# DavidBluecame/libYafaRay

Hardware: AMD Instinct MI355X
Metric: Mrays/sec + Msamples/sec, 1920×1080×64spp path-trace at 1/2/4/8 GPUs (higher is better)
Workload: dtype f32

## Files before the change

### libyafaray_amd/csrc/devscene.h

```cpp
#pragma once
#include <cstdint>
#include <hip/hip_runtime.h>

namespace yafamd
{
struct DevStats;

struct RadGrid
{
	const uint32_t *start;
	const float4 *pos;
	const float4 *dir;
	float lo[3];
	float cell, inv_cell;
	int nx, ny, nz;
};

enum : uint32_t
{
	B_NONE = 0, B_SPECULAR = 1u << 0, B_GLOSSY = 1u << 1, B_DIFFUSE = 1u << 2, B_DISPERSIVE = 1u << 3,
	B_REFLECT = 1u << 4, B_TRANSMIT = 1u << 5, B_FILTER = 1u << 6, B_EMIT = 1u << 7, B_VOLUMETRIC = 1u << 8,
	B_ALL = B_SPECULAR | B_GLOSSY | B_DIFFUSE | B_DISPERSIVE | B_REFLECT | B_TRANSMIT | B_FILTER
};

// ... 161 lines not shown
	float shadow_bias, ray_min_dist;
	uint32_t base_offset, rr_seed;
	float clamp_samples;
	int aa_multipass;
	uint32_t pass_offset;
	const uint32_t *plist;
	int nee_all_count;
	int faure_bytes;
	int small_tables;

	const float4 *ph_pos;
	const float4 *ph_dir;
	const float *ph_colb;
	const uint4 *pk_nodes;
	uint2 *pk_stack;
	int n_photons, pm_paths, pm_search, pm_stack;
	float pm_radius2;
	const int *ph_lights;
	const float *light_cdf;
	const float *light_func;
	float light_inv_integral;
	int n_ph_lights;
	const float4 *cph_pos;
	const float4 *cph_dir;
	const float *cph_colb;
	const uint4 *cpk_nodes;
	int caus_map, c_photons, c_paths, c_search;
	float c_radius2;
	int gather_on;
	int fg_on, fg_samples, fg_bounces;
	int fg_pass_samples;
	float fg_min_pathlen;
	float fg_lookup_rad;
	float fg_i_scale;
	const float4 *rph_pos;
	const float4 *rph_dir;
	const float *rph_colb;
	const uint4 *rpk_nodes;
	int n_rphotons;
	int rpk_lds;
	RadGrid rgrid;

	int has_attr, n_textures;
	const float4 *prim_attr;
	const float4 *texels;
	const DevTexture *textures;
	const DevNode *shader_nodes;

	int ext, tree, raydepth, cur_level;
	int max_add_depth;
	int bg_transp_refract;
	int tr_shad, s_depth;
	int do_ao, ao_samples;
	float ao_dist;
	float ao_col[3];
	struct DevStats *stats;
	int trace_stats;
	int crop_x0, crop_y0;
	int show_map;
	uint32_t node_base;
	uint32_t spawn_cap;
	float4 *node_own;
	int2 *node_child;
	float4 *node_w;
	float4 *spawn_o, *spawn_d;
	uint4 *spawn_pr;
	uint32_t *spawn_count;
	uint32_t *lpc;
	int lpc_mode;
	uint32_t *dfr_kind;
	float4 *dfr_pp;
	float4 *dfr_wo;
	float4 *dfr_a;
	float4 *dfr_emit;
	uint2 *dfr_pix;
	uint32_t *dfr_last;
	const uint32_t *dfr_seg_off;
	uint32_t dfr_cap;
	int nee_pm16;
	int w_live;
	int no_lean;
	int has_mesh_light;
	int fg_probe;
};

struct DevFilm
{
	float table[256];
	float filterw, table_scale;
	int reach_fwd, reach_back;
	int width, height, spp, tile;
	int multipass;
	uint32_t sample_offset;
	const uint32_t *tile_rank;
	int ntx;
	int partial;
	int crop_x0, crop_y0;
};

enum : int
{
	LK_BARYCENTRIC = 0, LK_DIFFUSE_COLOR, LK_MAT_INDEX_ABS, LK_MAT_INDEX_NORM, LK_MIST, LK_NORMAL_GEOM, LK_NORMAL_SMOOTH,
	LK_OBJ_INDEX_ABS, LK_OBJ_INDEX_NORM, LK_UV, LK_ZDEPTH_ABS, LK_ZDEPTH_NORM, LK_COUNT
};

struct DevLayers
{
	int n;
	int kind[LK_COUNT];
	const float4 *prim_attr;
	const float *mat_index;
	const int2 *obj_seg;
	int n_obj_seg;
	int n_prims, n_mats;
	float mat_highest, obj_highest;
	const float *depth;
	float4 *rec;
	float4 *albedo;
};

struct DevPaths
{
	float4 *thr;
	float4 *col;
	float4 *pcol;
	float4 *pwo;
	float4 *pend_thr;
	float4 *pend_emit;
	float4 *v0p;
	float4 *v0wo;
	uint4 *pr;
	float4 *csmp;
	float *nee;
	float *nee_aw;
	uint8_t *occ;
	float4 *ts;
	float4 *v0attr;
};

struct DevQueues
{
	int *slot;
	float *ray_o;
	float *ray_d;
	float2 *ray_tt;
	float tmin_dflt;
	float *hit_t;
	int *hit_prim;
	float4 *sh_o;
	float4 *sh_d;
	int *sh_idx;
	float2 *ts_hit;
	int *ts_n;
	float4 *sattr;
	const uint32_t *perm;
	int trace_part;
	int nee_grid;
};

enum : int
{
	TRACE_BOTH = 0,
	TRACE_CLOSEST = 1,
	TRACE_SHADOW = 2,
};

// ... 105 lines not shown
```

### libyafaray_amd/csrc/kernels.hip

```cpp

#include <hip/hip_runtime.h>
#include <cstdlib>
#include <string>
#include "devmath.h"
#include "photonheap.h"
#include "devscene.h"
#include "texeval.h"

namespace yafamd
{

#ifndef YAF_TRACE_BLOCK
#define YAF_TRACE_BLOCK 128
#endif
#ifndef YAF_SHADE_MIN_WAVES
#define YAF_SHADE_MIN_WAVES 4
#endif
#ifndef YAF_SHADE_LEAN_WAVES
#define YAF_SHADE_LEAN_WAVES 4
#endif
#ifndef YAF_SHADE_PREFETCH
#define YAF_SHADE_PREFETCH 1
#endif
constexpr int kTraceBlock = YAF_TRACE_BLOCK;
// ... 136 lines not shown
	__builtin_nontemporal_store(v, p);
#else
	*p = v;
#endif
}

__device__ __forceinline__ bool loadQRay(const DevQueues &Q, uint32_t i, V3 &o, V3 &d, float &tmin, float &tmax_w)
{
	const F3 dd = rayLd3(Q.ray_d, i);
	const F3 oo = rayLd3(Q.ray_o, i);
	d = v3(dd.x, dd.y, dd.z);
	o = v3(oo.x, oo.y, oo.z);
	if(dd.x != dd.x) return false;
	if(Q.ray_tt)
	{
		const float2 tt = Q.ray_tt[i];
		tmin = tt.x;
		tmax_w = tt.y;
	}
	else
	{
		tmin = Q.tmin_dflt;
		tmax_w = -1.f;
	}
	return true;
}
typedef float f32x3a4_t __attribute__((ext_vector_type(3))) __attribute__((aligned(4)));
__device__ __forceinline__ void storeQRay(const DevQueues &Q, uint32_t i, V3 o, V3 d)
{
#if YAF_NT_STORE2
	f32x3a4_t vo, vd;
	vo.x = o.x; vo.y = o.y; vo.z = o.z;
	vd.x = d.x; vd.y = d.y; vd.z = d.z;
	__builtin_nontemporal_store(vo, reinterpret_cast<f32x3a4_t *>(Q.ray_o + 3 * (size_t)i));
	__builtin_nontemporal_store(vd, reinterpret_cast<f32x3a4_t *>(Q.ray_d + 3 * (size_t)i));
#else
	reinterpret_cast<F3 *>(Q.ray_o)[i] = F3{o.x, o.y, o.z};
	reinterpret_cast<F3 *>(Q.ray_d)[i] = F3{d.x, d.y, d.z};
#endif
}
__device__ __forceinline__ void stStoreF3(float4 *base, uint32_t k, C3 c)
{
#if YAF_NT_STORE
	f32x3a4_t v;
	v.x = c.r; v.y = c.g; v.z = c.b;
	__builtin_nontemporal_store(v, reinterpret_cast<f32x3a4_t *>(reinterpret_cast<float *>(base) + 3 * (size_t)k));
#else
	reinterpret_cast<F3 *>(base)[k] = F3{c.r, c.g, c.b};
#endif
}
__device__ __forceinline__ void storeQNoRay(const DevQueues &Q, uint32_t i)
{
	Q.ray_d[3 * (size_t)i] = __builtin_nanf("");
}

constexpr uint32_t kPmSBits = 20, kPmLBits = 11;
__device__ __forceinline__ bool neePm8(const DevScene &S)
{
	return !S.nee_pm16 && (uint32_t)S.spp < (1u << kPmSBits) && S.n_lights <= (1 << kPmLBits);
}
typedef uint32_t u32x2_t __attribute__((ext_vector_type(2)));
#ifdef YAF_CHECKED
__device__ uint32_t g_nee_pm_err = 0;
#define NEE_PM_GUARD(cond) do { if(!(cond)) atomicCAS(&g_nee_pm_err, 0u, (uint32_t)__LINE__); } while(0)
#else
#define NEE_PM_GUARD(cond) do {} while(0)
#endif
__device__ __forceinline__ void neePmStore(const DevScene &S, uint4 *pm, uint32_t j, uint32_t offset, uint32_t sample_idx, uint32_t mode_l)
{
	if(neePm8(S))
	{
		NEE_PM_GUARD(sample_idx - S.base_offset - S.pass_offset < (uint32_t)S.spp);
		u32x2_t w;
		w.x = offset;
		w.y = (sample_idx - S.base_offset - S.pass_offset) | ((mode_l & 1u) << kPmSBits) | ((mode_l >> 8) << (kPmSBits + 1));
#if YAF_NT_STORE2
		__builtin_nontemporal_store(w, reinterpret_cast<u32x2_t *>(pm) + j);
#else
		reinterpret_cast<u32x2_t *>(pm)[j] = w;
#endif
	}
	else stStore2(&pm[j], make_uint4(offset, sample_idx, mode_l, 0u));
}
__device__ __forceinline__ uint4 neePmLoad(const DevScene &S, const uint4 *pm, uint32_t j)
{
	if(neePm8(S))
	{
		const uint2 w = reinterpret_cast<const uint2 *>(pm)[j];
		const uint32_t rel = w.y & ((1u << kPmSBits) - 1u);
		return make_uint4(w.x, S.base_offset + S.pass_offset + rel, ((w.y >> kPmSBits) & 1u) | ((w.y >> (kPmSBits + 1)) << 8), 0u);
	}
	return pm[j];
}

struct SegLoop
{
	uint32_t s, r, nb;
};
__device__ __forceinline__ SegLoop segLoop(uint32_t n_seg)
{
	SegLoop L;
	L.s = blockIdx.x % n_seg;
	L.r = blockIdx.x / n_seg;
	L.nb = (gridDim.x - L.s + n_seg - 1) / n_seg;
	return L;
}

#ifdef YAF_PHASE_TIMING
__device__ unsigned long long g_phase[16];
#define PHASE_DECL uint64_t ph_t = clock64(); uint64_t ph_acc[8] = {0, 0, 0, 0, 0, 0, 0, 0};
#define PHASE(k) do { const uint64_t t_ = clock64(); ph_acc[k] += t_ - ph_t; ph_t = t_; } while(0)
#define PHASE_FLUSH do { if(laneId() == 0) for(int k_ = 0; k_ < 8; ++k_) atomicAdd(&g_phase[k_], (unsigned long long)ph_acc[k_]); } while(0)
#else
#define PHASE_DECL
#define PHASE(k)
#define PHASE_FLUSH
#endif

struct SampleCoord { int x, y, s; };

__device__ SampleCoord sampleCoord(const DevJob *jobs, int n_jobs, int width, int tile, int spp, uint64_t sid)
{
	int j = 0, hi = n_jobs - 1;
	while(j < hi)
	{
		const int mid = (j + hi + 1) >> 1;
		if(jobs[mid].sample_base <= sid) j = mid;
		else hi = mid - 1;
	}
	const DevJob job = jobs[j];
	const uint64_t local = sid - job.sample_base;
	const uint32_t pix = (uint32_t)(local / (uint64_t)spp);
	const int s = (int)(local % (uint64_t)spp);
	const int bh = job.y1 - job.y0;
	const uint32_t per_tile = (uint32_t)(tile * bh);
	const int tx = (int)(pix / per_tile);
	const int tw = min(tile, width - tx * tile);
	const uint32_t l = pix - (uint32_t)tx * per_tile;
	SampleCoord c;
	c.x = tx * tile + (int)(l % (uint32_t)tw);
	c.y = job.y0 + (int)(l / (uint32_t)tw);
	c.s = s;
	return c;
}

__device__ __forceinline__ float biasDist(int bias, float r)
{
	if(bias == 1) return sqrtf(sqrtf(r) * r);
	if(bias == 2) return sqrtf(1.f - r * r);
	return sqrtf(r);
}

__device__ __forceinline__ void shirleyDisk(float r_1, float r_2, float &u, float &v)
{
	float phi = 0.f, r = 0.f;
	const float a = 2.f * r_1 - 1.f, b = 2.f * r_2 - 1.f;
	if(a > -b)
	{
		if(a > b) { r = a; phi = x87mul(kDivPiBy4, b / a); }
		else { r = b; phi = x87mul(kDivPiBy4, 2.f - a / b); }
	}
	else
	{
		if(a < b) { r = -a; phi = x87mul(kDivPiBy4, 4.f + b / a); }
		else
		{
			r = -b;
			phi = (b != 0) ? x87mul(kDivPiBy4, 6.f - a / b) : 0.f;
		}
	}
	u = r * fcos(phi);
	v = r * fsin(phi);
}

// ... 2028 lines not shown
}

__device__ __forceinline__ float ldsDim(const DevScene &S, int dim, uint32_t n)
{
	const uint4 fd = S.faure_dim[dim];
	UDiv dv;
	dv.m = fd.z;
	dv.sh = fd.w;
	return (float)lowDiscrepancy(S.faure + fd.y, fd.x, dv, S.faure_inv[dim], n);
}

__device__ __forceinline__ void copy16(uint4 *dst, const void *src, int n)
{
	const uint4 *s4 = reinterpret_cast<const uint4 *>(src);
	for(int k = threadIdx.x; k < n; k += blockDim.x) dst[k] = s4[k];
}

#ifndef YAF_STAGE_MATS
#define YAF_STAGE_MATS 1
#endif
constexpr size_t kStageMatsMax = 8192;
__host__ __device__ inline bool stageMatsOnly(const DevScene &S, bool small)
{
	return YAF_STAGE_MATS && !small && (size_t)S.n_mats * sizeof(DevMaterial) <= kStageMatsMax;
}
__host__ __device__ inline size_t shadeLdsBytes(const DevScene &S, bool small)
{
	size_t b = 50 * 16 + 25 * 16 + (size_t)S.faure_bytes;
	if(small) b += (size_t)S.n_mats * sizeof(DevMaterial) + (size_t)S.n_tris * 16;
	else if(stageMatsOnly(S, small)) b += (size_t)S.n_mats * sizeof(DevMaterial);
	return b;
}

template<bool SMALL>
__device__ __forceinline__ DevScene stageTables(const DevScene &G, uint4 *smem)
{
	DevScene S = G;
	uint4 *p = smem;
	copy16(p, G.faure_dim, 50);
	S.faure_dim = p;
	p += 50;
	copy16(p, G.faure_inv, 25);
	S.faure_inv = reinterpret_cast<const double *>(p);
	p += 25;
	if(SMALL)
	{
		const int nm = G.n_mats * (int)(sizeof(DevMaterial) / 16);
		copy16(p, G.mats, nm);
		S.mats = reinterpret_cast<const DevMaterial *>(p);
		p += nm;
		copy16(p, G.prim_ng, G.n_tris);
		S.prim_ng = reinterpret_cast<const float4 *>(p);
		p += G.n_tris;
	}
	else if(stageMatsOnly(G, false))
	{
		const int nm = G.n_mats * (int)(sizeof(DevMaterial) / 16);
		copy16(p, G.mats, nm);
		S.mats = reinterpret_cast<const DevMaterial *>(p);
		p += nm;
	}
	copy16(p, G.faure, G.faure_bytes / 16);
	S.faure = reinterpret_cast<const uint8_t *>(p);
	__syncthreads();
	return S;
}

struct ShadeArgs
{
	DevScene S;
	DevPaths Pc;
	DevPaths Pn;
	DevQueues Q;
	DevQueues Qn;
	DevNeeQueue N;
	DevNeeQueue G;
	DevCounters cnt;
	DevCounters cnt_next;
	float4 *samples;
	const DevJob *jobs;
	int n_jobs;
	uint64_t chunk_base;
};

__device__ __forceinline__ void writeSampleAt(const ShadeArgs &A, const SampleCoord &sc, C3 col, float alpha)
{
	if(alpha > 1.f) alpha = 1.f;
	A.samples[((size_t)sc.y * A.S.width + sc.x) * A.S.spp + sc.s] = f4(col, alpha);
}

__device__ __forceinline__ void writeSample(const ShadeArgs &A, uint32_t sid, C3 col, float alpha)
{
	writeSampleAt(A, sampleAt(A.S, A.jobs, A.n_jobs, A.chunk_base + (uint64_t)sid), col, alpha);
}

__device__ __forceinline__ Surf surfFromPrim(const DevScene &S, V3 p, int prim)
{
	Surf s;
	s.p = p;
	const float4 g = S.prim_ng[prim];
	s.ng = xyz(g);
	s.n = s.ng;
	coordsSystem(s.n, s.nu, s.nv);
	s.mat = __float_as_int(g.w);
	s.flags = S.mats[s.mat].bsdf_flags;
	const DevMaterial &m = S.mats[s.mat];
	s.dcol = C3{m.diffuse[0], m.diffuse[1], m.diffuse[2]};
	s.drefl = 1.f;
	s.sigma = 0.f;
	return s;
}

__device__ void spawnSpecular(const DevScene &S, const DevMaterial &m, const Surf &sp, V3 wo, uint32_t node, uint2 pix, uint2 rng,
                              int additional_depth)
{
	int2 child = make_int2(-1, -1);
	const int level = S.cur_level + 1;
	additional_depth = max(additional_depth, m.add_depth);
	if((sp.flags & (B_SPECULAR | B_FILTER)) && level <= S.raydepth + additional_depth && level < 20)
	{
		const SpecOut so = matSpecular(m, sp, wo);
		for(int k = 0; k < 2; ++k)
		{
			const bool want = k == 0 ? so.refl : so.refr;
			if(!want) continue;
			const uint32_t idx = atomicAdd(&S.spawn_count[0], 1u);
			if(idx >= S.spawn_cap) { atomicOr(&S.spawn_count[1], 1u); continue; }
			V3 from = sp.p;
			const V3 dir = k == 0 ? so.rdir : so.tdir;
			if(k == 1 && m.tbias > 0.f)
			{
				float f = m.tbias;
				if(m.sd_flags & SD_TBIAS_MULT) f *= (float)level;
				from = sp.p + dir * f;
			}
			S.spawn_o[idx] = f4(from, S.ray_min_dist);
			S.spawn_d[idx] = f4(dir, -1.f - (float)additional_depth);
			S.spawn_pr[idx] = make_uint4(pix.x, pix.y, rng.x ^ (0x9e3779b9u * (uint32_t)(2 * level + k + 1)), rng.y + 1u + (uint32_t)k);
			S.node_w[S.node_base + idx] = f4(k == 0 ? so.rcol : so.tcol, 0.f);
			if(k == 0) child.x = (int)(S.node_base + idx);
			else child.y = (int)(S.node_base + idx);
		}
	}
	S.node_child[node] = child;
}

template<bool SMALL, bool EXT, bool FUSED = false, bool LEAN = false, bool DEFER = false>
__global__ void __launch_bounds__(kShadeBlock, EXT ? 1 : (LEAN ? YAF_SHADE_LEAN_WAVES : YAF_SHADE_MIN_WAVES)) k_shade(ShadeArgs A)
{
	extern __shared__ uint4 shade_smem[];
	DevScene S_ = stageTables<SMALL>(A.S, shade_smem);
	if constexpr(LEAN)
	{
		S_.integrator = INT_PATH;
		S_.path_samples = 1;
		S_.do_ao = 0;
		S_.caus_map = 0;
		S_.show_map = 0;
		S_.gather_on = 0;
		S_.n_photons = 0;
		S_.fg_on = 0;
		S_.tree = 0;
		S_.has_attr = 0;
	}
	const DevScene S = S_;
	const bool ATTR = EXT && S.has_attr != 0;
// ... 755 lines not shown
			const uint32_t h = lo <= hi ? 1u : 0u;
			child[k] = __float_as_int(lane4(cf, k));
			const int count = __float_as_int(lane4(kf, k));
			const uint32_t inner = child[k] >= 0 ? 1u : 0u;
			key[k] = (h & inner) ? lo : inf;
			s4[k] = ~child[k] - acc;
			acc += (h & (inner ^ 1u)) ? count : 0;
			e4[k] = acc;
		}
		bool done = false;
		for(int i = 0; i < e4[3]; ++i)
		{
			const int q = i + (i < e4[0] ? s4[0] : i < e4[1] ? s4[1] : i < e4[2] ? s4[2] : s4[3]);
			if(STATS) TRACE_STAT(++tests);
			const float4 *tp = C.tris + 3 * q;
			const float4 ta = tp[0], tb = tp[1], tc = tp[2];
			const float t = triTest(ta, tb, tc, o, d, t_best);
			if(t == -1.f) continue;
			const int prim = __float_as_int(tb.w);
			if(any)
			{
				if(t < tmax && t >= 0.f) { t_best = t; prim_best = prim; done = true; break; }
			}
			else if(t >= tmin && (t < t_best || (t == t_best && prim_best >= 0 && prim < prim_best)))
			{
				t_best = t;
				prim_best = prim;
			}
		}
		if(!done)
		{
			cswap(key[0], child[0], key[1], child[1]);
			cswap(key[2], child[2], key[3], child[3]);
			cswap(key[0], child[0], key[2], child[2]);
			cswap(key[1], child[1], key[3], child[3]);
			cswap(key[1], child[1], key[2], child[2]);
			if(key[3] < inf) { C.stack[sp * STRIDE + lane] = child[3]; ++sp; }
			if(key[2] < inf) { C.stack[sp * STRIDE + lane] = child[2]; ++sp; }
			if(key[1] < inf) { C.stack[sp * STRIDE + lane] = child[1]; ++sp; }
			int next = key[0] < inf ? child[0] : -1;
			if(next < 0 && sp > 0)
			{
				--sp;
				next = C.stack[sp * STRIDE + lane];
			}
			node = next;
			done = next < 0;
		}
		if(done)
		{
			if(any) occ[cur] = prim_best >= 0 ? 1 : 0;
			else
			{
				hit_t = t_best;
				hit_prim = prim_best;
			}
			node = -1;
		}
	}
}

struct NeeArgs
{
	DevScene S;
	DevNeeQueue N;
	DevPaths Pn;
	DevQueues Qn;
	DevCounters cnt_next;
	int stack_depth;
};

__host__ __device__ inline size_t neeTraceLdsBytes(const DevScene &S, int stack_depth)
{
	return shadeLdsBytes(S, true) + (size_t)(S.node_f4 * S.n_nodes + 3 * S.n_tris) * 16 + (size_t)stack_depth * kShadeBlock * 4 +
	       (size_t)kShadeBlock * S.nee_k * 32;
}

#ifndef YAF_NEE_MIN_WAVES
#define YAF_NEE_MIN_WAVES 4
#endif
#ifndef YAF_NEE_LEAN_WAVES
#define YAF_NEE_LEAN_WAVES 4
#endif
#ifndef YAF_NEE_PREFETCH
#define YAF_NEE_PREFETCH 0
#endif
template<bool SMALL, bool EXT, bool TR = false, bool TSTATS = false, bool LEAN = false>
__global__ void __launch_bounds__(kShadeBlock, EXT ? 1 : (LEAN ? YAF_NEE_LEAN_WAVES : YAF_NEE_MIN_WAVES)) k_nee(NeeArgs A)
{
	extern __shared__ uint4 shade_smem[];
	DevScene S_ = stageTables<SMALL>(A.S, shade_smem);
	if constexpr(LEAN)
	{
		S_.do_ao = 0;
		S_.tr_shad = 0;
		S_.has_attr = 0;
	}
	const DevScene S = S_;
	const bool ATTR = EXT && S.has_attr != 0;
	TraceCtx C;
	C.wave_base = waveBase();
	float4 *rec = nullptr;
	if(TR)
	{
		float4 *lds_nodes = reinterpret_cast<float4 *>(shade_smem) + shadeLdsBytes(S, SMALL) / 16;
		float4 *lds_tris = lds_nodes + S.node_f4 * S.n_nodes;
		int *stack = reinterpret_cast<int *>(lds_tris + 3 * S.n_tris);
		rec = reinterpret_cast<float4 *>(stack + A.stack_depth * kShadeBlock) + 2 * threadIdx.x * S.nee_k;
		for(int k = threadIdx.x; k < S.node_f4 * S.n_nodes; k += blockDim.x) lds_nodes[k] = A.S.nodes[k];
		for(int k = threadIdx.x; k < 3 * S.n_tris; k += blockDim.x) lds_tris[k] = A.S.tris[k];
		__syncthreads();
		C.nodes = lds_nodes;
		C.tris = lds_tris;
		C.stack = stack;
		C.lds_depth = A.stack_depth;
		C.spill = nullptr;
		C.spill_stride = 0;
	}
	__shared__ uint32_t s_count;
	for(uint32_t seg = blockIdx.x; seg < S.n_seg; seg += gridDim.x)
	{
	uint32_t n_shadow = 0, n_dummy = 0, visits = 0, tests = 0;
	if(threadIdx.x == 0) s_count = 0;
	__syncthreads();
	ShadeOut out;
	out.sh_count = &s_count;
	out.sh_base = seg * S.cap_s;
	out.Qn = A.Qn;
	out.idx_in_o = !S.tr_shad;
	const uint32_t n_req = A.cnt_next.n_nee[seg];
	const uint32_t n_slots = A.cnt_next.n_active[seg];
	const uint32_t a0 = seg * S.cap_a;
	const int K = S.nee_k;
	const uint32_t stride = blockDim.x;
#if YAF_NEE_PREFETCH
	float4 wk_n = make_float4(0.f, 0.f, 0.f, 0.f);
	F3 o_n{0.f, 0.f, 0.f};
	uint4 pm_n = make_uint4(0u, 0u, 0u, 0u);
	if(threadIdx.x < n_slots)
	{
		wk_n = A.N.wo_k[a0 + threadIdx.x];
		o_n = reinterpret_cast<const F3 *>(A.Qn.ray_o)[a0 + threadIdx.x];
		pm_n = neePmLoad(S, A.N.pix_mode, a0 + threadIdx.x);
	}
#endif
	for(uint32_t base_j = 0; base_j < n_slots; base_j += stride)
	{
		const uint32_t j = a0 + base_j + threadIdx.x;
		float4 wk = make_float4(0.f, 0.f, 0.f, 0.f);
		V3 p = v3(0.f, 0.f, 0.f);
		uint4 pm = make_uint4(0u, 0u, 0u, 0u);
		bool live = base_j + threadIdx.x < n_slots;
#if YAF_NEE_PREFETCH
		if(live)
		{
			wk = wk_n;
			p = v3(o_n.x, o_n.y, o_n.z);
			pm = pm_n;
			live = !(wk.x != wk.x);
		}
		if(base_j + stride + threadIdx.x < n_slots)
		{
			wk_n = A.N.wo_k[j + stride];
			o_n = reinterpret_cast<const F3 *>(A.Qn.ray_o)[j + stride];
			pm_n = neePmLoad(S, A.N.pix_mode, j + stride);
		}
#else
		if(live)
		{
			wk = A.N.wo_k[j];
			const F3 o = reinterpret_cast<const F3 *>(A.Qn.ray_o)[j];
			p = v3(o.x, o.y, o.z);
			pm = neePmLoad(S, A.N.pix_mode, j);
			live = !(wk.x != wk.x);
		}
#endif
		Surf sp;
		sp.p = v3(0.f, 0.f, 0.f); sp.n = sp.ng = sp.nu = sp.nv = sp.p; sp.mat = 0; sp.flags = 0;
		sp.dcol = c3(0.f); sp.drefl = 1.f; sp.sigma = 0.f;
		if(live) sp = surfFromPrim(S, p, __float_as_int(wk.w));
		if(ATTR && live) applyAttr(sp, A.N.attr[2 * (size_t)j], A.N.attr[2 * (size_t)j + 1]);
		const V3 wo = xyz(wk);
		const int e0 = (int)j * K;
		const bool all = live && (pm.z & 1u);
		const bool one = live && !(pm.z & 1u);
		const uint32_t lnum = pm.z >> 8;
		if constexpr(TR)
		{
			if(live)
				for(int e = 0; e < K; ++e) rec[2 * e + 1] = make_float4(0.f, 0.f, 0.f, 0.f);
			const PathShadows rs{rec, e0};
			for(int l = 0; l < S.n_lights; ++l)
			{
				const bool mine = all || (one && lnum == (uint32_t)l);
				if(!__any(mine)) continue;
				neeLight<EXT>(S, S.lights[l], S.mats[sp.mat], sp, wo, (uint32_t)l, pm.y, pm.x, mine, e0 + (all ? (int)S.lights[l].nee_base : 0),
				              neeHbm(A.Pn), A.Pn.occ, rs);
			}
			float t_dummy;
			int p_dummy;
			if(__any(live))
				traceLaneRays<TSTATS, kShadeBlock>(C, rec, A.Pn.occ + e0, K, live, false, v3(0.f, 0.f, 0.f), v3(0.f, 0.f, 1.f), 0.f, 0.f, t_dummy,
				                                  p_dummy, visits, tests, n_dummy, n_shadow);
			continue;
		}
		if(__any(all))
		{
			for(int l = 0; l < S.n_lights; ++l)
				neeLight<EXT, ShadeOut, NeeHbm, LEAN>(S, S.lights[l], S.mats[sp.mat], sp, wo, (uint32_t)l, pm.y, pm.x, all,
				         e0 + (int)S.lights[l].nee_base, neeHbm(A.Pn), A.Pn.occ, out, S.tr_shad ? A.Pn.ts : nullptr);
			if(S.do_ao)
				aoSamples<EXT>(S, S.mats[sp.mat], sp, wo, pm.y, pm.x, all, e0 + S.nee_all_count, neeHbm(A.Pn), A.Pn.occ, out,
				               S.tr_shad ? A.Pn.ts : nullptr);
		}
		if(__any(one))
		{
			for(int l = 0; l < S.n_lights; ++l)
			{
				const bool mine = one && lnum == (uint32_t)l;
				if(!__any(mine)) continue;
				neeLight<EXT, ShadeOut, NeeHbm, LEAN>(S, S.lights[l], S.mats[sp.mat], sp, wo, (uint32_t)l, pm.y, pm.x, mine, e0, neeHbm(A.Pn), A.Pn.occ, out,
				              S.tr_shad ? A.Pn.ts : nullptr);
			}
		}
	}
	if(TR)
	{
		for(int off = 32; off > 0; off >>= 1) n_shadow += __shfl_down(n_shadow, off);
		if(laneId() == 0 && n_shadow) atomicAdd(&s_count, n_shadow);
	}
	__syncthreads();
	if(threadIdx.x == 0)
	{
		A.cnt_next.n_shadow[seg] = TR ? 0u : s_count;
		if(S.stats)
		{
			S.stats[seg].nee_requests += n_req;
			if(TR) S.stats[seg].shadow_rays += s_count;
		}
	}
	if(TR && TSTATS && S.stats)
	{
		for(int off = 32; off > 0; off >>= 1)
		{
			visits += __shfl_down(visits, off);
			tests += __shfl_down(tests, off);
		}
		if(laneId() == 0)
		{
			atomicAdd(&S.stats[seg].node_visits, (unsigned long long)visits);
			atomicAdd(&S.stats[seg].tri_tests, (unsigned long long)tests);
		}
	}
	}
}

struct DfrArgs
{
	DevScene S;
// ... 2721 lines not shown
					if(v.w != 0.f) path_col = path_col + rgb(v);
				}
			}
		}
		const C3 fg = path_col / (float)B.n_sampl;
		const uint4 cb = A.G.pix_mode[j];
		const C3 col = C3{__uint_as_float(cb.x), __uint_as_float(cb.y), __uint_as_float(cb.z)} + fg;
		A.G.pix_mode[j] = make_uint4(__float_as_uint(col.r), __float_as_uint(col.g), __float_as_uint(col.b), cb.w);
	}
}

}

using namespace yafamd;

extern "C" {

int yafamd_trace_block() { return kTraceBlock; }

int yafamd_shade_fused() { return kShadeFused ? 1 : 0; }
int yafamd_shade_fused_for(const DevScene *S)
{
	if(S->ext) return 0;
	if(kShadeFused) return 1;
	return (YAF_FUSE_LEAN && S->integrator == INT_PATH && S->path_samples <= 1 && !S->do_ao && !S->caus_map && !S->gather_on && !S->show_map &&
	        S->n_photons == 0 && !S->tree && !S->has_attr && !S->no_lean && !S->tr_shad && !S->has_mesh_light) ? 1 : 0;
}

int yafamd_experiments() { return kExperiments ? 1 : 0; }

#ifndef YAF_DEVICE_BUILD
#define YAF_DEVICE_BUILD "arch=? extra=[?] (built outside csrc/Makefile)"
#endif
const char *yafamd_device_build() { return YAF_DEVICE_BUILD
#ifdef YAF_PHASE_TIMING
	" phase-timing"
#endif
	; }

int yafamd_phase_cycles(unsigned long long *out, int n, int reset)
{
#ifdef YAF_PHASE_TIMING
	unsigned long long h[16];
	if(hipMemcpyFromSymbol(h, HIP_SYMBOL(g_phase), sizeof(h)) != hipSuccess) return 0;
	for(int k = 0; k < n && k < 16; ++k) out[k] = h[k];
	if(reset)
	{
		const unsigned long long z[16] = {};
		if(hipMemcpyToSymbol(HIP_SYMBOL(g_phase), z, sizeof(z)) != hipSuccess) return 0;
	}
	return 16;
#else
	(void)out; (void)n; (void)reset;
	return 0;
#endif
}

int yafamd_trace_blocks_per_cu(int lds_scene, int wide, size_t dyn_lds)
{
	int nb = 0;
	hipError_t e;
	if(wide == 8) e = hipOccupancyMaxActiveBlocksPerMultiprocessor(&nb, k_trace<false, true, false, true, false, false, true>, kTraceBlock, dyn_lds);
	else if(lds_scene) e = wide ? hipOccupancyMaxActiveBlocksPerMultiprocessor(&nb, k_trace<true, true, false>, kTraceBlock, dyn_lds)
	                       : hipOccupancyMaxActiveBlocksPerMultiprocessor(&nb, k_trace<true, false, false>, kTraceBlock, dyn_lds);
	else e = wide ? hipOccupancyMaxActiveBlocksPerMultiprocessor(&nb, k_trace<false, true, false>, kTraceBlock, dyn_lds)
	              : hipOccupancyMaxActiveBlocksPerMultiprocessor(&nb, k_trace<false, false, false>, kTraceBlock, dyn_lds);
	return e == hipSuccess ? nb : 0;
}

int yafamd_path_blocks_per_cu(const DevScene *S, int stack_depth)
{
	int nb = 0;
#ifdef YAF_EXPERIMENTS
	if(hipOccupancyMaxActiveBlocksPerMultiprocessor(&nb, k_path<false>, kTraceBlock, pathLdsBytes(*S, stack_depth)) != hipSuccess) nb = 0;
#else
	(void)S; (void)stack_depth;
#endif
	return nb;
}

int yafamd_nee_blocks_per_cu()
{
	int nb = 0;
	if(hipOccupancyMaxActiveBlocksPerMultiprocessor(&nb, (k_nee<true, false>), kShadeBlock, 8192) != hipSuccess) nb = 0;
	return nb;
}

int yafamd_shade_blocks_per_cu()
{
	int nb = 0;
	if(hipOccupancyMaxActiveBlocksPerMultiprocessor(&nb, (k_shade<true, false>), kShadeBlock, 8192) != hipSuccess) nb = 0;
	return nb;
}

hipError_t yafamd_launch_camera(const DevScene *S, const DevPaths *P, const DevQueues *Q, const DevCounters *cnt,
                                const DevJob *jobs, int n_jobs, uint64_t chunk_base, int n, hipStream_t st)
{
	if(n <= 0) return hipSuccess;
	const int threads = max(n, (int)S->n_seg);
	hipLaunchKernelGGL(k_camera, dim3((threads + 255) / 256), dim3(256), 0, st, *S, *P, *Q, *cnt, jobs, n_jobs, chunk_base, n);
	return hipGetLastError();
}

hipError_t yafamd_launch_trace(const DevScene *S, const DevQueues *Q, const DevCounters *cnt, const DevPaths *P,
                               DevStats *stats, int stack_depth, int *spill, int grid, hipStream_t st)
{
	const size_t stack_bytes = (size_t)stack_depth * kTraceBlock * sizeof(int);
	const bool wide = S->node_f4 == 8;
	const size_t lds_scene = S->scene_in_lds ? (size_t)(S->node_f4 * S->n_nodes + 3 * S->n_tris) * sizeof(float4)
	                                         : (wide ? (size_t)S->lds_top * kTopStride * sizeof(float4) : 0);
	const size_t bytes = stack_bytes + lds_scene;
	if(S->nodes8 && !S->scene_in_lds && !S->tr_shad)
	{
		const size_t bytes8 = stack_bytes + (size_t)S->lds_top8 * kTop8Stride * sizeof(float4);
		if(S->trace_stats)
			hipLaunchKernelGGL((k_trace<false, true, false, true, true, false, true>), dim3(grid), dim3(kTraceBlock), bytes8, st, *S, *Q, *cnt, *P, stats,
			                   stack_depth, spill);
		else
			hipLaunchKernelGGL((k_trace<false, true, false, true, false, false, true>), dim3(grid), dim3(kTraceBlock), bytes8, st, *S, *Q, *cnt, *P, stats,
			                   stack_depth, spill);
		return hipGetLastError();
	}
#ifdef YAF_EXPERIMENTS
	if(S->brute && !S->tr_shad && S->n_tris <= kBruteTris)
	{
		hipLaunchKernelGGL(k_trace_brute, dim3(grid), dim3(kTraceBlock), 0, st, *S, *Q, *cnt, *P, stats);
		return hipGetLastError();
	}
#endif
#define YAF_TRACE_LAUNCH(L, W, T, SP) hipLaunchKernelGGL((k_trace<L, W, T, SP>), dim3(grid), dim3(kTraceBlock), bytes, st, *S, *Q, *cnt, *P, stats, stack_depth, spill)
	const bool nospill = spill == nullptr;
	if(S->tr_shad)
	{
		if(S->scene_in_lds)
		{
			if(nospill) { if(wide) YAF_TRACE_LAUNCH(true, true, true, false); else YAF_TRACE_LAUNCH(true, false, true, false); }
			else if(wide) YAF_TRACE_LAUNCH(true, true, true, true);
			else YAF_TRACE_LAUNCH(true, false, true, true);
		}
		else if(wide) YAF_TRACE_LAUNCH(false, true, true, true);
		else YAF_TRACE_LAUNCH(false, false, true, true);
	}
	else if(S->scene_in_lds)
	{
#ifdef YAF_EXPERIMENTS
		if(nospill && wide && S->ray_sort)
		{
			if(S->trace_stats)
				hipLaunchKernelGGL((k_trace<true, true, false, false, true, true>), dim3(grid), dim3(kTraceBlock), bytes, st, *S, *Q, *cnt, *P, stats,
				                   stack_depth, spill);
			else
				hipLaunchKernelGGL((k_trace<true, true, false, false, false, true>), dim3(grid), dim3(kTraceBlock), bytes, st, *S, *Q, *cnt, *P, stats,
				                   stack_depth, spill);
		}
		else
#endif
		if(nospill && wide && !S->trace_stats)
			hipLaunchKernelGGL((k_trace<true, true, false, false, false>), dim3(grid), dim3(kTraceBlock), bytes, st, *S, *Q, *cnt, *P, stats,
			                   stack_depth, spill);
		else if(nospill) { if(wide) YAF_TRACE_LAUNCH(true, true, false, false); else YAF_TRACE_LAUNCH(true, false, false, false); }
		else if(wide) YAF_TRACE_LAUNCH(true, true, false, true);
		else YAF_TRACE_LAUNCH(true, false, false, true);
	}
#ifdef YAF_EXPERIMENTS
	else if(wide && S->ray_sort)
	{
		if(S->trace_stats)
// ... 143 lines not shown
}

hipError_t yafamd_launch_surface(const DevScene *S, const DevQueues *Q, const DevCounters *cnt, hipStream_t st)
{
	hipLaunchKernelGGL(k_surface, dim3(S->n_seg), dim3(kShadeBlock), 0, st, *S, *Q, *cnt);
	return hipGetLastError();
}

hipError_t yafamd_launch_tshadow(const DevScene *S, const DevQueues *Q, const DevCounters *cnt, const DevPaths *P, hipStream_t st)
{
	hipLaunchKernelGGL(k_tshadow, dim3(S->n_seg), dim3(kShadeBlock), 0, st, *S, *Q, *cnt, *P);
	return hipGetLastError();
}

int yafamd_path_eligible(const DevScene *S, int stack_depth, int spill)
{
	return (kExperiments && !S->ext && !S->tree && !S->tr_shad && !S->has_attr && !S->do_ao && !S->gather_on && !S->caus_map && S->integrator != INT_PHOTON &&
	        S->scene_in_lds && S->node_f4 == 8 && !spill && S->small_tables && S->nee_k >= 1 && S->nee_k <= kPathMaxK && !S->brute &&
	        pathLdsBytes(*S, stack_depth) <= 64 * 1024)
	           ? 1
	           : 0;
}

hipError_t yafamd_launch_path(const DevScene *S, float4 *samples, const DevJob *jobs, int n_jobs, uint64_t chunk_base, uint32_t n,
                              uint32_t *next, int stack_depth, int grid, hipStream_t st)
{
	if(!yafamd_path_eligible(S, stack_depth, 0)) return hipErrorInvalidValue;
	if(n == 0) return hipSuccess;
	PathArgs A;
	A.S = *S;
	A.samples = samples;
	A.jobs = jobs;
	A.n_jobs = n_jobs;
	A.chunk_base = chunk_base;
	A.n = n;
	A.next = next;
	A.stack_depth = stack_depth;
#ifdef YAF_EXPERIMENTS
	const size_t lds = pathLdsBytes(*S, stack_depth);
	if(S->trace_stats) hipLaunchKernelGGL(k_path<true>, dim3(grid), dim3(kTraceBlock), lds, st, A);
	else hipLaunchKernelGGL(k_path<false>, dim3(grid), dim3(kTraceBlock), lds, st, A);
	return hipGetLastError();
#else
	(void)grid; (void)st;
	return hipErrorInvalidValue;
#endif
}

int yafamd_nee_trace_eligible(const DevScene *S, int stack_depth)
{
	return (kExperiments && !S->ext && !S->tr_shad && !S->has_attr && S->scene_in_lds && S->node_f4 == 8 && S->small_tables && S->nee_k >= 1 &&
	        S->nee_k <= kPathMaxK && !S->brute && neeTraceLdsBytes(*S, stack_depth) <= 64 * 1024)
	           ? 1
	           : 0;
}

hipError_t yafamd_launch_nee(const DevScene *S, const DevNeeQueue *N, const DevPaths *Pn, const DevQueues *Qn,
                             const DevCounters *cnt_next, int stack_depth, hipStream_t st)
{
	NeeArgs A;
	A.S = *S;
	A.N = *N;
	A.Pn = *Pn;
	A.Qn = *Qn;
	A.cnt_next = *cnt_next;
	const size_t lds = shadeLdsBytes(*S, S->small_tables != 0);
	A.stack_depth = stack_depth;
	const int grid = (Qn->nee_grid > 0 && Qn->nee_grid < (int)S->n_seg) ? Qn->nee_grid : (int)S->n_seg;
#ifdef YAF_EXPERIMENTS
	if(stack_depth > 0 && yafamd_nee_trace_eligible(S, stack_depth))
	{
		if(S->trace_stats) hipLaunchKernelGGL((k_nee<true, false, true, true>), dim3(grid), dim3(kShadeBlock), neeTraceLdsBytes(*S, stack_depth), st, A);
		else hipLaunchKernelGGL((k_nee<true, false, true>), dim3(grid), dim3(kShadeBlock), neeTraceLdsBytes(*S, stack_depth), st, A);
		return hipGetLastError();
	}
#endif
	if(S->ext)
	{
		if(S->small_tables) hipLaunchKernelGGL((k_nee<true, true>), dim3(grid), dim3(kShadeBlock), lds, st, A);
		else hipLaunchKernelGGL((k_nee<false, true>), dim3(grid), dim3(kShadeBlock), lds, st, A);
	}
	else if(!S->do_ao && !S->tr_shad && !S->has_mesh_light && !S->no_lean)
	{
		if(S->small_tables) hipLaunchKernelGGL((k_nee<true, false, false, false, true>), dim3(grid), dim3(kShadeBlock), lds, st, A);
		else hipLaunchKernelGGL((k_nee<false, false, false, false, true>), dim3(grid), dim3(kShadeBlock), lds, st, A);
	}
	else if(S->small_tables) hipLaunchKernelGGL((k_nee<true, false>), dim3(grid), dim3(kShadeBlock), lds, st, A);
	else hipLaunchKernelGGL((k_nee<false, false>), dim3(grid), dim3(kShadeBlock), lds, st, A);
	return hipGetLastError();
}

hipError_t yafamd_photon_emit(const DevScene *S, const PhotonState *P, const PhotonSet *L, uint32_t n_photons, uint32_t h0, uint32_t n_local,
                              int max_bounces, hipStream_t st)
{
	PhotonArgs A;
	A.S = *S;
	A.P = *P;
	A.L = *L;
	A.n_photons = n_photons;
	A.h0 = h0;
	A.n_local = n_local;
	A.max_bounces = max_bounces;
	A.bounce = 0;
	A.cur = 0;
	A.stack_depth = 0;
	A.spill = nullptr;
	if(n_local == 0) return hipSuccess;
	hipLaunchKernelGGL(k_photon_emit, dim3((n_local + 255) / 256), dim3(256), 0, st, A);
	return hipGetLastError();
}

hipError_t yafamd_photon_bounce(const DevScene *S, const PhotonState *P, const PhotonSet *L, uint32_t n_photons, uint32_t h0,
                                uint32_t n_local, int max_bounces, int bounce, int cur, int stack_depth, int *spill, int grid, hipStream_t st)
{
	PhotonArgs A;
	A.S = *S;
	A.P = *P;
	A.L = *L;
	A.n_photons = n_photons;
	A.h0 = h0;
	A.n_local = n_local;
	A.max_bounces = max_bounces;
	A.bounce = bounce;
	A.cur = cur;
	A.stack_depth = stack_depth;
	A.spill = spill;
	if((uint32_t)grid != P->n_segs) return hipErrorInvalidValue;
	const size_t stack_bytes = (size_t)stack_depth * kTraceBlock * sizeof(int);
	if(S->scene_in_lds)
	{
		const size_t bytes = stack_bytes + (size_t)(S->node_f4 * S->n_nodes + 3 * S->n_tris) * sizeof(float4);
		const bool ns = spill == nullptr;
		if(S->ext)
		{
			if(S->node_f4 == 8)
			{
				if(ns) hipLaunchKernelGGL((k_photon_bounce<true, true, true, false>), dim3(grid), dim3(kTraceBlock), bytes, st, A);
				else hipLaunchKernelGGL((k_photon_bounce<true, true, true>), dim3(grid), dim3(kTraceBlock), bytes, st, A);
			}
			else hipLaunchKernelGGL((k_photon_bounce<true, false, true>), dim3(grid), dim3(kTraceBlock), bytes, st, A);
		}
		else if(S->node_f4 == 8)
		{
			if(ns) hipLaunchKernelGGL((k_photon_bounce<true, true, false, false>), dim3(grid), dim3(kTraceBlock), bytes, st, A);
			else hipLaunchKernelGGL((k_photon_bounce<true, true, false>), dim3(grid), dim3(kTraceBlock), bytes, st, A);
		}
		else hipLaunchKernelGGL((k_photon_bounce<true, false, false>), dim3(grid), dim3(kTraceBlock), bytes, st, A);
	}
	else if(S->ext)
	{
		if(S->node_f4 == 8) hipLaunchKernelGGL((k_photon_bounce<false, true, true>), dim3(grid), dim3(kTraceBlock), stack_bytes, st, A);
		else hipLaunchKernelGGL((k_photon_bounce<false, false, true>), dim3(grid), dim3(kTraceBlock), stack_bytes, st, A);
	}
	else if(S->node_f4 == 8) hipLaunchKernelGGL((k_photon_bounce<false, true, false>), dim3(grid), dim3(kTraceBlock), stack_bytes, st, A);
	else hipLaunchKernelGGL((k_photon_bounce<false, false, false>), dim3(grid), dim3(kTraceBlock), stack_bytes, st, A);
	return hipGetLastError();
}

hipError_t yafamd_photon_compact(const PhotonState *P, uint32_t *scratch_counts, uint32_t *total_dev, float4 *pos, float4 *dir, float *colb,
                                 hipStream_t st)
{
	const uint32_t nb = (P->n_local + 1023u) / 1024u;
	if(nb == 0) return hipSuccess;
	hipLaunchKernelGGL(k_photon_count, dim3(nb), dim3(256), 0, st, P->dep_flag, P->n_local, P->n_slot_rows, scratch_counts);
	hipLaunchKernelGGL(k_photon_scan, dim3(1), dim3(1024), 0, st, scratch_counts, nb, total_dev);
	hipLaunchKernelGGL(k_photon_scatter, dim3(nb), dim3(1024), 0, st, *P, (const uint32_t *)scratch_counts, pos, dir, colb);
	return hipGetLastError();
// ... 264 lines not shown
```

### libyafaray_amd/csrc/render.cc

```cpp
#include "render.h"
#include "devmath.h"
#include "photonfile.h"

#include <hip/hip_runtime.h>
#include <rccl/rccl.h>

#include <algorithm>
#include <array>
#include <chrono>
#include <cmath>
#include <cstdlib>
#include <cstring>
#include <future>
#include <mutex>
#include <sstream>
#include <unordered_map>

using namespace yafamd;

extern "C" {
hipError_t yafamd_launch_camera(const DevScene *S, const DevPaths *P, const DevQueues *Q, const DevCounters *cnt,
                                const DevJob *jobs, int n_jobs, uint64_t chunk_base, int n, hipStream_t st);
hipError_t yafamd_launch_surface(const DevScene *S, const DevQueues *Q, const DevCounters *cnt, hipStream_t st);
hipError_t yafamd_launch_tshadow(const DevScene *S, const DevQueues *Q, const DevCounters *cnt, const DevPaths *P, hipStream_t st);
// ... 1999 lines not shown
			const char *we = std::getenv("YAFARAY_AMD_GATHER_WALK");
			const uint32_t exact = (yafamd_experiments() && we && std::string(we) == "bound") ? 0u : 1u;
			glog = GatherLogDesc{d.g_log.p, (uint32_t *)d.g_log_n.p, cap, (uint32_t)seg_cap, 0u, split, exact, nullptr};
			const int lv = yafamd_walk_lds_levels(d.pm_stack), deep = std::max(1, d.pm_stack) - lv;
			if(deep > 0)
			{
				if(!ensure(log_, d.walk_spill, (size_t)deep * yafamd_walk_threads(&S) * 4)) return false;
				glog.spill = (uint32_t *)d.walk_spill.p;
			}
			walk_gather = true;
		}
	}
	const bool fg_paths = yafamd_fg_paths_eligible(&S) != 0;
	bool ray_bin = false;
	if(const char *e = std::getenv("YAFARAY_AMD_RAY_BIN"); e && *e == '1' && S.nodes8 && !S.scene_in_lds && !S.tr_shad && R <= 1024)
	{
		const size_t n = (size_t)R * S.cap_a;
		size_t tb = 0;
		HIPCHECK(yafamd_ray_bin(nullptr, nullptr, (uint32_t)R, S.cap_a, nullptr, nullptr, nullptr, nullptr, nullptr, nullptr, nullptr, &tb, d.stream));
		if(!ensure(log_, d.bin_keys, n * 4) || !ensure(log_, d.bin_keys2, n * 4) || !ensure(log_, d.bin_iota, n * 4) || !ensure(log_, d.bin_perm, n * 4) ||
		   !ensure(log_, d.bin_tmp, tb))
			return false;
		ray_bin = true;
	}
	FgBatch fgb{};
	auto fgPrepare = [&]() -> bool {
		const int ns = S.fg_pass_samples > 0 ? S.fg_pass_samples : std::max(1, S.fg_samples);
		const int nt = std::max(0, S.fg_bounces) + 1;
		const size_t per_pos = (size_t)R * (size_t)ns * (16 + 48 + 16 * (size_t)nt);
		size_t cap_max = std::max<size_t>(1, ((size_t)6 << 30) / per_pos);
		if(const char *e = getenv("YAFARAY_AMD_FG_BATCH"); e && atoi(e) > 0) cap_max = std::min(cap_max, (size_t)atoi(e));
		const size_t nb = ((size_t)S.cap_a + cap_max - 1) / cap_max;
		const size_t seg_cap = std::max<size_t>(1, ((size_t)S.cap_a + nb - 1) / std::max<size_t>(1, nb));
		const size_t paths = (size_t)R * seg_cap * (size_t)ns;
		if(!ensure(log_, d.fg_terms, paths * 16) || !ensure(log_, d.fg_longs, paths * 48) || !ensure(log_, d.fg_long_terms, paths * 16 * (size_t)nt) ||
		   !ensure(log_, d.fg_long_count, (size_t)R * 4))
			return false;
		fgb = FgBatch{0u, (uint32_t)seg_cap, ns, nt, (float4 *)d.fg_terms.p, (float4 *)d.fg_longs.p, (float4 *)d.fg_long_terms.p,
		              (uint32_t *)d.fg_long_count.p, (uint32_t)(seg_cap * (size_t)ns)};
		return true;
	};
	if(!ensure(log_, d.counters, 2 * 4 * R * sizeof(uint32_t))) return false;
	if(!ensure(log_, d.stats, sizeof(DevStats) * 2 * (size_t)d.trace_grid)) return false;
	HIPCHECK(hipMemsetAsync(d.counters.p, 0, 2 * 4 * R * sizeof(uint32_t), d.stream));
	HIPCHECK(hipMemsetAsync(d.stats.p, 0, sizeof(DevStats) * 2 * (size_t)d.trace_grid, d.stream));
	DevCounters cnt[2];
	for(int q = 0; q < 2; ++q)
	{
		uint32_t *base_q = (uint32_t *)d.counters.p + (size_t)q * 4 * R;
		cnt[q].n_active = base_q;
		cnt[q].n_shadow = base_q + R;
		cnt[q].n_nee = base_q + 2 * R;
		cnt[q].n_gather = base_q + 3 * R;
	}
	DevStats *dstats = (DevStats *)d.stats.p;
	S.stats = dstats;
	int nee_trace_stack = 0;
	{
		const char *ne = std::getenv("YAFARAY_AMD_NEE_TRACE");
		if(yafamd_experiments() && ne && std::string(ne) == "1" && d.lds_stack >= d.stack_depth) nee_trace_stack = d.lds_stack;
	}
	bool overlap = rp.device_sharers <= 1;
	int ov_nee_grid = std::max(1, (int)S.n_seg / 2), ov_trace_grid = std::max((int)S.n_seg, std::min(2 * (int)S.n_seg, d.trace_grid));
	if(const char *e = std::getenv("YAFARAY_AMD_OVERLAP"); e && *e) overlap = *e != '0';
	if(const char *e = std::getenv("YAFARAY_AMD_OVERLAP_NEE_GRID"); e && atoi(e) > 0) ov_nee_grid = atoi(e);
	if(const char *e = std::getenv("YAFARAY_AMD_OVERLAP_TRACE_GRID"); e && atoi(e) > 0)
		ov_trace_grid = (int)S.n_seg * std::max(1, std::min(atoi(e), d.trace_grid) / (int)S.n_seg);
	overlap = overlap && S.scene_in_lds && !S.ray_sort && !S.brute && !ray_bin && !S.tree && !S.tr_shad && !S.has_attr && nee_trace_stack == 0;
	bool ov_shadow = true;
	int ov_shadow_grid = d.trace_grid;
	if(const char *e = std::getenv("YAFARAY_AMD_OVERLAP_SHADOW"); e && *e) ov_shadow = *e != '0';
	if(const char *e = std::getenv("YAFARAY_AMD_OVERLAP_SHADOW_GRID"); e && atoi(e) > 0)
		ov_shadow_grid = (int)S.n_seg * std::max(1, std::min(atoi(e), d.trace_grid) / (int)S.n_seg);
	ov_shadow = ov_shadow && overlap && d.spill.p == nullptr;
	bool lpc_on = S.integrator == INT_PATH && S.n_lights > 1 && !S.tree && (rp.shard_world <= 1 || group_render);
	if(const char *lp = std::getenv("YAFARAY_AMD_LIGHT_PICK"); lp && std::string(lp) == "hash") lpc_on = false;
	lpc_carry_ = 0;
	S.lpc = nullptr;
	S.lpc_mode = 0;
	S.nee_pm16 = 0;
	if(const char *e = std::getenv("YAFARAY_AMD_NEE_PM16"); e && *e == '1') S.nee_pm16 = 1;
	if(const char *e = std::getenv("YAFARAY_AMD_W_LIVE"); e && *e == '1') S.w_live = 1;
	S.no_lean = 0;
	S.fg_probe = 0;
	if(const char *e = std::getenv("YAFARAY_AMD_FG_PROBE"); e && *e) S.fg_probe = atoi(e);
	if(const char *e = std::getenv("YAFARAY_AMD_SHADE_LEAN"); e && *e == '0') S.no_lean = 1;
	int path_grid = 0;
	if(!lpc_on)
	{
		const char *pe = std::getenv("YAFARAY_AMD_PATH");
		const bool on = yafamd_experiments() && pe && std::string(pe) == "mega";
		if(on && yafamd_path_eligible(&S, d.lds_stack, d.lds_stack < d.stack_depth ? 1 : 0))
		{
			path_grid = std::min(d.trace_grid, d.n_cu * std::max(1, yafamd_path_blocks_per_cu(&S, d.lds_stack)));
			if(const char *e = getenv("YAFARAY_AMD_PATH_GRID")) path_grid = std::min(d.trace_grid, std::max(1, atoi(e)));
			if(!ensure(log_, d.path_next, 16)) return false;
		}
	}
	const int n_paths = std::max(1, S.path_samples);
	const int iters = (S.integrator == INT_PATH) ? 2 + n_paths * (S.bounces + 2) : 3;

	auto ensureEvents = [&](size_t need) -> bool {
		while(d.ev_pool.size() < need)
		{
			hipEvent_t e;
			HIPCHECK(hipEventCreate(&e));
			d.ev_pool.push_back(e);
		}
		return true;
	};
	if(!ensureEvents(2)) return false;
	HIPCHECK(hipEventRecord(d.ev_pool[0], d.stream));
	DevStats *run_stats = dstats;
	auto iterate = [&](uint64_t base) -> bool {
		int cur = 0;
		const bool count_run = S.lpc_mode == 1;
		bool closest_done = false;
		for(int it = 0; it < iters; ++it)
		{
			DevQueues qc = d.Q[cur];
			if(it != 0 || (S.cur_level == 0 && !S.cam.ray_tt)) qc.ray_tt = nullptr;
			qc.tmin_dflt = it == 0 ? 0.f : S.ray_min_dist;
			qc.perm = nullptr;
			qc.trace_part = closest_done ? TRACE_SHADOW : TRACE_BOTH;
			const bool join_pending = closest_done && ov_shadow;
			closest_done = false;
			if(ray_bin && it >= 1 && !count_run)
			{
				size_t tb = d.bin_tmp.bytes;
				HIPCHECK(yafamd_ray_bin(&qc, &cnt[cur], S.n_seg, S.cap_a, d.scene_lo, d.scene_hi, (uint32_t *)d.bin_keys.p, (uint32_t *)d.bin_keys2.p,
				                        (uint32_t *)d.bin_iota.p, (uint32_t *)d.bin_perm.p, d.bin_tmp.p, &tb, d.stream));
				qc.perm = (const uint32_t *)d.bin_perm.p;
			}
			if(join_pending)
			{
				bool ok = [&]() -> bool {
					PROF(KK_TRACE, yafamd_launch_trace(&S, &qc, &cnt[cur], &d.P[cur], run_stats + d.trace_grid, d.lds_stack, nullptr, ov_shadow_grid,
					                                    d.stream));
					HIPCHECK(hipStreamWaitEvent(d.stream, d.ev_join, 0));
					return true;
				}();
				if(!ok)
				{
					(void)hipStreamSynchronize(d.side);
					return false;
				}
			}
			else
				PROF(KK_TRACE, yafamd_launch_trace(&S, &qc, &cnt[cur], &d.P[cur], run_stats, d.lds_stack, (int *)d.spill.p,
				                                    S.tr_shad ? d.trace_grid_bvh4 : d.trace_grid, d.stream));
			if(S.tr_shad && !count_run) PROF(KK_TSHADOW, yafamd_launch_tshadow(&S, &qc, &cnt[cur], &d.P[cur], d.stream));
			if(S.has_attr) PROF(KK_SURFACE, yafamd_launch_surface(&S, &qc, &cnt[cur], d.stream));
			if(S.lpc_mode == 3)
				HIPCHECK(yafamd_dfr_segoff(&cnt[cur], S.n_seg, (uint32_t *)d.dfr_segoff.p, (uint32_t *)d.dfr_misc.p, S.dfr_cap,
				                           (uint32_t *)d.dfr_misc.p + 1, (uint32_t *)d.dfr_its.p, d.stream));
			PROF(KK_SHADE, yafamd_launch_shade(&S, &d.P[cur], &d.P[cur ^ 1], &qc, &d.Q[cur ^ 1], &d.N, &d.G, &cnt[cur], &cnt[cur ^ 1],
			                             (float4 *)d.samples.p, (const DevJob *)d.jobs.p, n_jobs, base, d.stream));

			const bool dl_pipeline = S.integrator != INT_PATH;
			if(S.gather_on && !count_run && (!dl_pipeline || it == 1 || (S.show_map && it == 0)))
			{
				if(S.fg_on && fg_paths)
				{
					if(!fgPrepare()) return false;
					for(uint32_t j0 = 0; j0 < S.cap_a; j0 += fgb.seg_cap)
					{
// ... 981 lines not shown
```

Before: 2169.

## Prefetch NEE slot inputs into LDS via global_load_lds DMA in lean k_nee

Replaces the compile-time register prefetch in the lean NEE kernel with an asynchronous global-to-LDS DMA prefetch (global_load_lds) of wo_k, ray origins and pixel-mode words for the next iteration. Each wave gets a 3 KB LDS staging area, and the loads for iteration j+stride are issued while the current slot is shaded, so global latency is hidden without holding extra registers. This costs 6 KB more LDS per block, which may lower occupancy. The path is on by default and can be turned off with an environment variable.

```diff
diff --git a/libyafaray_amd/csrc/devscene.h b/libyafaray_amd/csrc/devscene.h
--- a/libyafaray_amd/csrc/devscene.h
+++ b/libyafaray_amd/csrc/devscene.h
@@ -267,6 +267,7 @@
 	int no_lean;
 	int has_mesh_light;
 	int fg_probe;
+	int nee_pf_lds;
 };
 
 struct DevFilm
diff --git a/libyafaray_amd/csrc/kernels.hip b/libyafaray_amd/csrc/kernels.hip
--- a/libyafaray_amd/csrc/kernels.hip
+++ b/libyafaray_amd/csrc/kernels.hip
@@ -242,14 +242,14 @@
 	}
 	else stStore2(&pm[j], make_uint4(offset, sample_idx, mode_l, 0u));
 }
+__device__ __forceinline__ uint4 neePmWide(const DevScene &S, uint2 w)
+{
+	const uint32_t rel = w.y & ((1u << kPmSBits) - 1u);
+	return make_uint4(w.x, S.base_offset + S.pass_offset + rel, ((w.y >> kPmSBits) & 1u) | ((w.y >> (kPmSBits + 1)) << 8), 0u);
+}
 __device__ __forceinline__ uint4 neePmLoad(const DevScene &S, const uint4 *pm, uint32_t j)
 {
-	if(neePm8(S))
-	{
-		const uint2 w = reinterpret_cast<const uint2 *>(pm)[j];
-		const uint32_t rel = w.y & ((1u << kPmSBits) - 1u);
-		return make_uint4(w.x, S.base_offset + S.pass_offset + rel, ((w.y >> kPmSBits) & 1u) | ((w.y >> (kPmSBits + 1)) << 8), 0u);
-	}
+	if(neePm8(S)) return neePmWide(S, reinterpret_cast<const uint2 *>(pm)[j]);
 	return pm[j];
 }
 
@@ -2444,6 +2444,22 @@
 	int n_jobs;
 	uint64_t chunk_base;
 };
+
+template<int SIZE>
+__device__ __forceinline__ void ldsDma(const void *src, char *wave_dst)
+{
+	static_assert(SIZE == 4 || SIZE == 12 || SIZE == 16, "global_load_lds_dword / x3 / x4");
+	const auto *g = (const __attribute__((address_space(1))) void *)src;
+	auto *l = (__attribute__((address_space(3))) void *)wave_dst;
+	if constexpr(SIZE == 4) __builtin_amdgcn_global_load_lds(g, l, 4, 0, 0);
+	else if constexpr(SIZE == 12) __builtin_amdgcn_global_load_lds(g, l, 12, 0, 0);
+	else __builtin_amdgcn_global_load_lds(g, l, 16, 0, 0);
+}
+__device__ __forceinline__ void ldsDmaLanded() { asm volatile("s_waitcnt vmcnt(0)" ::: "memory"); }
+__device__ __forceinline__ void ldsReadsRetired() { asm volatile("s_waitcnt lgkmcnt(0)" ::: "memory"); }
+constexpr uint32_t kPfPitch12 = 16;
+constexpr uint32_t kNeePfWk = 0, kNeePfO = 1024, kNeePfPm = 2048, kNeePfWave = 3072;
+constexpr size_t kNeePfBytes = (size_t)(kShadeBlock / 64) * kNeePfWave;
 
 __device__ __forceinline__ void writeSampleAt(const ShadeArgs &A, const SampleCoord &sc, C3 col, float alpha)
 {
@@ -3365,12 +3381,10 @@
 #ifndef YAF_NEE_LEAN_WAVES
 #define YAF_NEE_LEAN_WAVES 4
 #endif
-#ifndef YAF_NEE_PREFETCH
-#define YAF_NEE_PREFETCH 0
-#endif
-template<bool SMALL, bool EXT, bool TR = false, bool TSTATS = false, bool LEAN = false>
+template<bool SMALL, bool EXT, bool TR = false, bool TSTATS = false, bool LEAN = false, bool PFL = false>
 __global__ void __launch_bounds__(kShadeBlock, EXT ? 1 : (LEAN ? YAF_NEE_LEAN_WAVES : YAF_NEE_MIN_WAVES)) k_nee(NeeArgs A)
 {
+	static_assert(!PFL || (LEAN && !EXT && !TR), "PFL: the lean k_nee");
 	extern __shared__ uint4 shade_smem[];
 	DevScene S_ = stageTables<SMALL>(A.S, shade_smem);
 	if constexpr(LEAN)
@@ -3401,6 +3415,21 @@
 		C.spill_stride = 0;
 	}
 	__shared__ uint32_t s_count;
+	char *const pf = reinterpret_cast<char *>(shade_smem) + shadeLdsBytes(A.S, SMALL) + (threadIdx.x >> 6) * kNeePfWave;
+	const uint32_t pf_lane = threadIdx.x & 63u;
+	const bool pm8 = neePm8(S);
+	auto pfIssue = [&](uint32_t e, bool on) {
+		if(!on) return;
+		ldsDma<16>(A.N.wo_k + e, pf + kNeePfWk);
+		ldsDma<12>(A.Qn.ray_o + 3 * (size_t)e, pf + kNeePfO);
+		if(pm8)
+		{
+			const uint32_t *w = reinterpret_cast<const uint32_t *>(reinterpret_cast<const uint2 *>(A.N.pix_mode) + e);
+			ldsDma<4>(w, pf + kNeePfPm);
+			ldsDma<4>(w + 1, pf + kNeePfPm + 256);
+		}
+		else ldsDma<16>(A.N.pix_mode + e, pf + kNeePfPm);
+	};
 	for(uint32_t seg = blockIdx.x; seg < S.n_seg; seg += gridDim.x)
 	{
 	uint32_t n_shadow = 0, n_dummy = 0, visits = 0, tests = 0;
@@ -3416,17 +3445,11 @@
 	const uint32_t a0 = seg * S.cap_a;
 	const int K = S.nee_k;
 	const uint32_t stride = blockDim.x;
-#if YAF_NEE_PREFETCH
-	float4 wk_n = make_float4(0.f, 0.f, 0.f, 0.f);
-	F3 o_n{0.f, 0.f, 0.f};
-	uint4 pm_n = make_uint4(0u, 0u, 0u, 0u);
-	if(threadIdx.x < n_slots)
-	{
-		wk_n = A.N.wo_k[a0 + threadIdx.x];
-		o_n = reinterpret_cast<const F3 *>(A.Qn.ray_o)[a0 + threadIdx.x];
-		pm_n = neePmLoad(S, A.N.pix_mode, a0 + threadIdx.x);
-	}
-#endif
+	if constexpr(PFL)
+	{
+		ldsReadsRetired();
+		pfIssue(a0 + threadIdx.x, threadIdx.x < n_slots);
+	}
 	for(uint32_t base_j = 0; base_j < n_slots; base_j += stride)
 	{
 		const uint32_t j = a0 + base_j + threadIdx.x;
@@ -3434,21 +3457,24 @@
 		V3 p = v3(0.f, 0.f, 0.f);
 		uint4 pm = make_uint4(0u, 0u, 0u, 0u);
 		bool live = base_j + threadIdx.x < n_slots;
-#if YAF_NEE_PREFETCH
-		if(live)
-		{
-			wk = wk_n;
-			p = v3(o_n.x, o_n.y, o_n.z);
-			pm = pm_n;
-			live = !(wk.x != wk.x);
-		}
-		if(base_j + stride + threadIdx.x < n_slots)
-		{
-			wk_n = A.N.wo_k[j + stride];
-			o_n = reinterpret_cast<const F3 *>(A.Qn.ray_o)[j + stride];
-			pm_n = neePmLoad(S, A.N.pix_mode, j + stride);
-		}
-#else
+		if constexpr(PFL)
+		{
+			ldsDmaLanded();
+			if(live)
+			{
+				wk = *reinterpret_cast<const float4 *>(pf + kNeePfWk + 16u * pf_lane);
+				const float *o = reinterpret_cast<const float *>(pf + kNeePfO + kPfPitch12 * pf_lane);
+				p = v3(o[0], o[1], o[2]);
+				const uint32_t *w = reinterpret_cast<const uint32_t *>(pf + kNeePfPm);
+				if(pm8) pm = neePmWide(S, make_uint2(w[pf_lane], w[64u + pf_lane]));
+				else pm = *reinterpret_cast<const uint4 *>(pf + kNeePfPm + 16u * pf_lane);
+				live = !(wk.x != wk.x);
+			}
+			ldsReadsRetired();
+			pfIssue(j + stride, base_j + stride + threadIdx.x < n_slots);
+		}
+		else
+		{
 		if(live)
 		{
 			wk = A.N.wo_k[j];
@@ -3457,7 +3483,7 @@
 			pm = neePmLoad(S, A.N.pix_mode, j);
 			live = !(wk.x != wk.x);
 		}
-#endif
+		}
 		Surf sp;
 		sp.p = v3(0.f, 0.f, 0.f); sp.n = sp.ng = sp.nu = sp.nv = sp.p; sp.mat = 0; sp.flags = 0;
 		sp.dcol = c3(0.f); sp.drefl = 1.f; sp.sigma = 0.f;
@@ -6345,7 +6371,7 @@
 int yafamd_nee_blocks_per_cu()
 {
 	int nb = 0;
-	if(hipOccupancyMaxActiveBlocksPerMultiprocessor(&nb, (k_nee<true, false>), kShadeBlock, 8192) != hipSuccess) nb = 0;
+	if(hipOccupancyMaxActiveBlocksPerMultiprocessor(&nb, (k_nee<true, false>), kShadeBlock, 8192 + kNeePfBytes) != hipSuccess) nb = 0;
 	return nb;
 }
 
@@ -6655,7 +6681,13 @@
 	}
 	else if(!S->do_ao && !S->tr_shad && !S->has_mesh_light && !S->no_lean)
 	{
-		if(S->small_tables) hipLaunchKernelGGL((k_nee<true, false, false, false, true>), dim3(grid), dim3(kShadeBlock), lds, st, A);
+		if(S->nee_pf_lds)
+		{
+			if(S->small_tables)
+				hipLaunchKernelGGL((k_nee<true, false, false, false, true, true>), dim3(grid), dim3(kShadeBlock), lds + kNeePfBytes, st, A);
+			else hipLaunchKernelGGL((k_nee<false, false, false, false, true, true>), dim3(grid), dim3(kShadeBlock), lds + kNeePfBytes, st, A);
+		}
+		else if(S->small_tables) hipLaunchKernelGGL((k_nee<true, false, false, false, true>), dim3(grid), dim3(kShadeBlock), lds, st, A);
 		else hipLaunchKernelGGL((k_nee<false, false, false, false, true>), dim3(grid), dim3(kShadeBlock), lds, st, A);
 	}
 	else if(S->small_tables) hipLaunchKernelGGL((k_nee<true, false>), dim3(grid), dim3(kShadeBlock), lds, st, A);
diff --git a/libyafaray_amd/csrc/render.cc b/libyafaray_amd/csrc/render.cc
--- a/libyafaray_amd/csrc/render.cc
+++ b/libyafaray_amd/csrc/render.cc
@@ -2105,6 +2105,8 @@
 	if(const char *e = std::getenv("YAFARAY_AMD_NEE_PM16"); e && *e == '1') S.nee_pm16 = 1;
 	if(const char *e = std::getenv("YAFARAY_AMD_W_LIVE"); e && *e == '1') S.w_live = 1;
 	S.no_lean = 0;
+	S.nee_pf_lds = 1;
+	if(const char *e = std::getenv("YAFARAY_AMD_NEE_PREFETCH"); e && *e) S.nee_pf_lds = std::string(e) == "lds" ? 1 : 0;
 	S.fg_probe = 0;
 	if(const char *e = std::getenv("YAFARAY_AMD_FG_PROBE"); e && *e) S.fg_probe = atoi(e);
 	if(const char *e = std::getenv("YAFARAY_AMD_SHADE_LEAN"); e && *e == '0') S.no_lean = 1;
```

New measurement: 2177, median of 6. About the same (+0.4%).
